# thomaspingel/neilpy

Hardware: AMD Instinct MI355X
Metric: Mcells/s through SMRF progressive_filter, 16384x16384 fp32 DEM (higher is better)
Workload: dtype f32

## Files before the change

include/smrf_hip.h:

```cpp
#ifndef SMRF_HIP_H
#define SMRF_HIP_H

#include <stddef.h>
#include <stdint.h>

#ifdef __cplusplus
extern "C" {
#endif

#define SMRF_ABI_VERSION 1

#if defined(__GNUC__)
#define SMRF_API __attribute__((visibility("default")))
#else
#define SMRF_API
#endif

#define SMRF_OK 0
#define SMRF_E_ARG (-1)
#define SMRF_E_HIP (-2)
#define SMRF_E_WORKSPACE (-3)
#define SMRF_E_RANGE (-4)
#define SMRF_E_UNSUPPORTED (-5)

// ... 46 lines not shown
SMRF_API size_t smrf_progressive_filter_workspace_bytes(int rows, int cols, int elem_size);
SMRF_API int smrf_progressive_filter_f32(const float* d_Z, int rows, int cols, const int32_t* h_windows,
                                const double* h_thresholds, int n_windows, uint8_t* d_mask,
                                uint8_t* d_when_dropped, void* d_workspace,
                                size_t workspace_bytes, int nan_aware, int impl, void* stream);
SMRF_API int smrf_progressive_filter_f64(const double* d_Z, int rows, int cols, const int32_t* h_windows,
                                const double* h_thresholds, int n_windows, uint8_t* d_mask,
                                uint8_t* d_when_dropped, void* d_workspace,
                                size_t workspace_bytes, int nan_aware, int impl, void* stream);

#define SMRF_ROUTE_TWO_PASS 0
#define SMRF_ROUTE_FUSED 1
#define SMRF_ROUTE_DIRECT 2
#define SMRF_ROUTE_COPY 3
#define SMRF_ROUTE_CHAIN 4
SMRF_API int smrf_progressive_filter_timed_f32(const float* d_Z, int rows, int cols, const int32_t* h_windows,
                                const double* h_thresholds, int n_windows, uint8_t* d_mask,
                                uint8_t* d_when_dropped, void* d_workspace, size_t workspace_bytes, int nan_aware,
                                int impl, void* stream, float* h_window_ms, int32_t* h_window_route);
SMRF_API int smrf_progressive_filter_timed_f64(const double* d_Z, int rows, int cols, const int32_t* h_windows,
                                const double* h_thresholds, int n_windows, uint8_t* d_mask,
                                uint8_t* d_when_dropped, void* d_workspace, size_t workspace_bytes, int nan_aware,
                                int impl, void* stream, float* h_window_ms, int32_t* h_window_route);

SMRF_API int smrf_count_nan_f32(const float* d_a, int64_t n, int64_t* h_count, void* stream);
SMRF_API int smrf_count_nan_f64(const double* d_a, int64_t n, int64_t* h_count, void* stream);

SMRF_API int smrf_points_extent_f64(const double* d_x, const double* d_y, int64_t n, double* h_out,
                           void* d_workspace, size_t workspace_bytes, void* stream);
SMRF_API int smrf_las_decode_xyz_f64(const uint8_t* d_records, int64_t npts, int record_length,
                            const double* h_scale_offset, double* d_x, double* d_y, double* d_z,
                            void* stream);
SMRF_API int smrf_affine_apply_f64(const double* d_x, const double* d_y, int64_t npts, const double* h_inv,
                          double* d_col, double* d_row, void* stream);
SMRF_API int smrf_grid_clear_u64(uint64_t* d_keys, int64_t ncells, void* stream);
SMRF_API int smrf_grid_bin_f64(const double* d_x, const double* d_y, const double* d_z, int64_t npts,
                      const double* h_inv, const double* h_filter, uint64_t* d_keys,
                      int rows_total, int cols, int row0, int rows_local, int is_max,
                      int64_t* d_n_outside, void* stream);
SMRF_API int smrf_grid_finalize_f64(const uint64_t* d_keys, double* d_grid, uint8_t* d_empty,
                           int64_t ncells, int is_max, void* stream);

SMRF_API int smrf_points_band_count_f64(const double* d_x, const double* d_y, int64_t npts, const double* h_inv,
                               int rows_total, int nbands, uint64_t* d_counts, void* stream);
SMRF_API int smrf_points_band_pack_f64(const double* d_x, const double* d_y, const double* d_z, int64_t npts,
                              const double* h_inv, int rows_total, int nbands, uint64_t* d_cursors,
// ... 92 lines not shown
```

neilpy_amd/_lib.py:

```python
import ctypes as C
import os

_HERE = os.path.dirname(os.path.abspath(__file__))
LIB_PATH = os.environ.get("NEILPY_AMD_LIB") or os.path.join(_HERE, "_lib", "libsmrf_hip.so")

IMPL_AUTO, IMPL_RING, IMPL_DIRECT = 0, 1, 2
ROUTE_TWO_PASS, ROUTE_FUSED, ROUTE_DIRECT, ROUTE_COPY, ROUTE_CHAIN = 0, 1, 2, 3, 4
RING_MAX_RADIUS = 64
TERRAIN_IMPL_AUTO, TERRAIN_IMPL_TILED, TERRAIN_IMPL_DIRECT = 0, 1, 2
TERRAIN_HALO_CAP = {"f32": 40, "f64": 24}
TERRAIN_OPENNESS, TERRAIN_SKYVIEW, TERRAIN_COUNT, TERRAIN_TERNARY = 0, 1, 2, 3
(SURFACE_SLOPE, SURFACE_ASPECT, SURFACE_HILLSHADE, SURFACE_HORN, SURFACE_LAPLACE, SURFACE_ESRI, SURFACE_ZT,
 SURFACE_EVANS, SURFACE_WG) = range(9)
SURFACE_OPT_RADIANS, SURFACE_OPT_DEGREES = 1, 2


class SmrfHipError(RuntimeError):
    pass


_p = C.c_void_p
_i = C.c_int
_i64 = C.c_int64
_d = C.c_double
_sz = C.c_size_t

SIGNATURES = {
    "smrf_abi_version": (_i, []),
    "smrf_last_error": (C.c_char_p, []),
    "smrf_device_count": (_i, []),
    "smrf_switches_reload": (None, []),
    "smrf_disk_filter_f32": (_i, [_p, _p, _i, _i, _i64, _i, _i, _i, _i, _i, _i, _i, _i, _p]),
    "smrf_disk_filter_f64": (_i, [_p, _p, _i, _i, _i64, _i, _i, _i, _i, _i, _i, _i, _i, _p]),
    "smrf_pf_dilate_flag_f32": (_i, [_p, _p, _p, _p, _p, _d, _i, _i, _i, _i64, _i, _i, _i, _i, _i, _i, _i, _p]),
    "smrf_pf_dilate_flag_f64": (_i, [_p, _p, _p, _p, _p, _d, _i, _i, _i, _i64, _i, _i, _i, _i, _i, _i, _i, _p]),
    "smrf_fused_open_supported": (_i, [_i, _i]),
    "smrf_pf_open_flag_f32": (_i, [_p, _p, _p, _p, _d, _i, _i, _i, _i64, _i, _i, _i, _i, _i, _p]),
    "smrf_pf_open_flag_f64": (_i, [_p, _p, _p, _p, _d, _i, _i, _i, _i64, _i, _i, _i, _i, _i, _p]),
    "smrf_pf_chain_length": (_i, [_i, _p, _i, _i64]),
    "smrf_pf_chain_flag_f32": (_i, [_p, _p, _p, _p, _p, _p, _p, _i, _i, _i, _i64, _i, _i, _i, _i, _p]),
    "smrf_pf_chain_flag_f64": (_i, [_p, _p, _p, _p, _p, _p, _p, _i, _i, _i, _i64, _i, _i, _i, _i, _p]),
    "smrf_progressive_filter_workspace_bytes": (_sz, [_i, _i, _i]),
    "smrf_progressive_filter_f32": (_i, [_p, _i, _i, _p, _p, _i, _p, _p, _p, _sz, _i, _i, _p]),
    "smrf_progressive_filter_f64": (_i, [_p, _i, _i, _p, _p, _i, _p, _p, _p, _sz, _i, _i, _p]),
    "smrf_progressive_filter_timed_f32": (_i, [_p, _i, _i, _p, _p, _i, _p, _p, _p, _sz, _i, _i, _p, _p, _p]),
    "smrf_progressive_filter_timed_f64": (_i, [_p, _i, _i, _p, _p, _i, _p, _p, _p, _sz, _i, _i, _p, _p, _p]),
    "smrf_count_nan_f32": (_i, [_p, _i64, C.POINTER(_i64), _p]),
    "smrf_count_nan_f64": (_i, [_p, _i64, C.POINTER(_i64), _p]),
    "smrf_points_extent_f64": (_i, [_p, _p, _i64, C.POINTER(_d), _p, _sz, _p]),
    "smrf_las_decode_xyz_f64": (_i, [_p, _i64, _i, C.POINTER(_d), _p, _p, _p, _p]),
    "smrf_affine_apply_f64": (_i, [_p, _p, _i64, C.POINTER(_d), _p, _p, _p]),
    "smrf_points_band_count_f64": (_i, [_p, _p, _i64, C.POINTER(_d), _i, _i, _p, _p]),
    "smrf_points_band_pack_f64": (_i, [_p, _p, _p, _i64, C.POINTER(_d), _i, _i, _p, _p, _p, _p, _p]),
    "smrf_grid_clear_u64": (_i, [_p, _i64, _p]),
    "smrf_grid_bin_f64": (_i, [_p, _p, _p, _i64, C.POINTER(_d), C.POINTER(_d), _p, _i, _i, _i, _i, _i, _p, _p]),
    "smrf_grid_finalize_f64": (_i, [_p, _p, _p, _i64, _i, _p]),
    "smrf_springs_workspace_bytes": (_sz, [_i, _i]),
    "smrf_springs_lsqr_f64": (_i, [_p, _i, _i, _d, _d, _d, _i64, C.POINTER(_i), C.POINTER(_i64),
                                   C.POINTER(_i64), _p, _sz, _p]),
    "smrf_fda_workspace_bytes": (_sz, [_i, _i]),
    "smrf_fda_lsqr_f64": (_i, [_p, _i, _i, _d, _d, _d, _i64, C.POINTER(_i), C.POINTER(_i64),
                               C.POINTER(_i64), _p, _sz, _p]),
    "smrf_fda_apply_f64": (_i, [_p, _i, _i, _p, _p, _p, _p, _p, _p, _p, _sz, _p]),
    "smrf_springs_band_workspace_bytes": (_sz, [_i, _i]),
    "smrf_springs_band_layout": (_i, [_i, _i, C.POINTER(_i64)]),
    "smrf_springs_band_begin": (_i, [_i, _i, _d, _d, _d, _i64, _p, _sz, _p]),
    "smrf_springs_band_phase": (_i, [_i, _p, _i, _i, _i, _i, _p, _sz, _p]),
    "smrf_springs_band_status": (_i, [_p, _i, _i, C.POINTER(_i), C.POINTER(_i64), C.POINTER(_i64), C.POINTER(_i), _p]),
    "smrf_gradient_slope_f64": (_i, [_p, _p, _i, _i, _d, _p]),
# ... 56 lines not shown
```

neilpy_amd/build.py:

```python
import argparse
import os
import shutil
import subprocess
import sys
from concurrent.futures import ThreadPoolExecutor

PKG = os.path.dirname(os.path.abspath(__file__))
ROOT = os.path.dirname(PKG)
CSRC = os.path.join(PKG, "csrc")
OBJ = os.path.join(PKG, "_build")
LIBDIR = os.path.join(PKG, "_lib")
LIB = os.path.join(LIBDIR, "libsmrf_hip.so")
RING_PARTS = 8

FLAGS = ["-std=c++20", "-O3", "--offload-arch=gfx950", "-fPIC", "-ffp-contract=off",
         "-fvisibility=hidden", "-Wall", "-Wno-unused-function",
         "-I" + os.path.join(ROOT, "include"), "-I" + CSRC]


def hipcc():
    exe = shutil.which("hipcc") or "/opt/rocm/bin/hipcc"
    if not os.path.exists(exe):
        raise RuntimeError("hipcc not found: libsmrf_hip cannot be built (there is no CPU fallback)")
    return exe


def units():
    out = [(n + ".o", os.path.join(CSRC, n + ".hip"), []) for n in ("core", "morph", "chain", "grid", "springs", "fda", "tail", "spline", "terrain", "surface")]
    for f64 in (0, 1):
        for p in range(RING_PARTS):
            out.append(("ring_%s_p%d.o" % ("f64" if f64 else "f32", p), os.path.join(CSRC, "ring_part.hip"),
                        ["-DPART=%d" % p, "-DSMRF_F64=%d" % f64]))
    return out


def newest_header():
    t = os.path.getmtime(os.path.join(ROOT, "include", "smrf_hip.h"))
    for f in os.listdir(CSRC):
        if f.endswith((".h", ".inc")):
            t = max(t, os.path.getmtime(os.path.join(CSRC, f)))
    return t


def build(jobs=None, force=False, verbose=True, variant=None, defs=()):
    global OBJ, LIB
    if variant:
        OBJ = os.path.join(PKG, "_build", "variant_" + variant)
        LIB = os.path.join(LIBDIR, "variants", variant + ".so")
        os.makedirs(os.path.dirname(LIB), exist_ok=True)
    os.makedirs(OBJ, exist_ok=True)
    os.makedirs(LIBDIR, exist_ok=True)
# ... 46 lines not shown
```

neilpy_amd/csrc/core.hip:

```cpp
#include <atomic>
#include <cstring>

#include "smrf_common.h"

namespace {
thread_local char g_err[512] = "";
}

namespace {
int env_int(const char* name, int dflt) {
  const char* v = getenv(name);
  return v && *v ? atoi(v) : dflt;
}
SmrfSwitches read_switches() {
  SmrfSwitches s;
  s.fused = env_int("SMRF_FUSED", 1);
  s.chain = env_int("SMRF_CHAIN", 1);
  s.nan_ride = env_int("SMRF_NAN_RIDE", 1);
  s.nt = env_int("SMRF_NT", -1);
  s.ring_seg = env_int("SMRF_RING_SEG", 0);
  s.ring_dual = env_int("SMRF_RING_DUAL", -1);
  s.ring_rounds = env_int("SMRF_RING_ROUNDS", 1);
  s.ring_slope = env_int("SMRF_RING_SLOPE", -1);
  s.seg_rule = env_int("SMRF_SEG_RULE", 0);
  s.xcd_remap = env_int("SMRF_XCD_REMAP", 1);
  s.fused_rounds = env_int("SMRF_FUSED_ROUNDS", 1);
  s.chain_rounds = env_int("SMRF_CHAIN_ROUNDS", 3);
  s.ring_debug = env_int("SMRF_RING_DEBUG", 0);
  return s;
}
std::atomic<const SmrfSwitches*> g_sw{new SmrfSwitches(read_switches())};
}

const SmrfSwitches& smrf_sw() { return *g_sw.load(std::memory_order_acquire); }

int smrf_fail(int code, const char* fmt, ...) {
  va_list ap;
  va_start(ap, fmt);
  vsnprintf(g_err, sizeof(g_err), fmt, ap);
  va_end(ap);
  return code;
}

extern "C" {

int smrf_abi_version(void) { return SMRF_ABI_VERSION; }

const char* smrf_last_error(void) { return g_err; }

void smrf_switches_reload(void) { g_sw.store(new SmrfSwitches(read_switches()), std::memory_order_release); }

// ... 11 lines not shown
```

neilpy_amd/csrc/morph.hip:

```cpp
#include <algorithm>
#include <cmath>
#include <cstdlib>
#include <cstring>
#include <vector>

#include "smrf_common.h"
#include "morph_chain.h"

namespace {

template <typename T>
__device__ __forceinline__ void flag_cell(const DiskArgs<T>& a, long long off, T lastval, T val) {
  const T diff = lastval - val;
  bool hit;
  if constexpr (sizeof(T) == 4) hit = diff > a.thr_lo;
  else hit = (double)diff > a.thr;
  if (a.dense) {
    a.mask[off] = hit ? 1 : 0;
    if (a.when != nullptr) a.when[off] = hit ? (uint8_t)a.widx : (uint8_t)0;
  } else if (hit) {
    a.mask[off] = 1;
    if (a.when != nullptr) a.when[off] = (uint8_t)a.widx;
  }
}
// ... 208 lines not shown
  if (!last || !opened || !mask || !radii || !thr || !widx) return smrf_fail(SMRF_E_ARG, "null pointer");
  if (n < 1 || n > 4) return smrf_fail(SMRF_E_ARG, "a chain has 1..4 windows (got %d)", n);
  const int pat = smrf_chain_match((int)sizeof(T), radii, n, 1ll << 62);
  if (pat < 0 || smrf_chain_length(pat) != n)
    return smrf_fail(SMRF_E_UNSUPPORTED, "no chained launch for these %d radii at this dtype (smrf_pf_chain_length tells)", n);
  DiskArgs<T> b{};
  b.in = last; b.out = opened; b.img_rows = img_rows; b.cols = cols; b.ld = ld;
  b.in_row0 = in_row0; b.in_rows = in_rows; b.out_row0 = out_row0; b.out_rows = out_rows;
  b.radius = smrf_chain_halo(pat);
  if (int rc = check_band(b)) return rc;
  if (b.radius >= img_rows) return smrf_fail(SMRF_E_UNSUPPORTED, "raster of %d rows is shorter than the chain's %d halo rows", img_rows, b.radius);
  ChainArgs<T> c{};
  c.in = last; c.out = opened; c.mask = mask; c.when = when;
  for (int k = 0; k < n; ++k) { c.thr[k] = thr[k]; c.widx[k] = widx[k]; }
  c.img_rows = img_rows; c.cols = cols; c.ld = ld;
  c.in_row0 = in_row0; c.in_rows = in_rows; c.out_row0 = out_row0; c.out_rows = out_rows;
  c.seg = smrf_sw().ring_seg;
  c.nt = nt_rule<T>(img_rows, cols);
  c.dense0 = 0;
  if constexpr (sizeof(T) == 4) return smrf_chain_f32(pat, c, (hipStream_t)stream);
  else return smrf_chain_f64(pat, c, (hipStream_t)stream);
}

template <typename T>
int progressive_filter_api(const T* Z, int rows, int cols, const int32_t* windows, const double* thr, int nwin,
                           uint8_t* mask, uint8_t* when, void* ws, size_t ws_bytes, int nan_aware, int impl,
                           void* stream_, float* h_window_ms = nullptr, int32_t* h_window_route = nullptr) {
  hipStream_t stream = (hipStream_t)stream_;
  if (!Z || !mask || (nwin > 0 && (!windows || !thr))) return smrf_fail(SMRF_E_ARG, "null pointer");
  if (rows < 1 || cols < 1 || nwin < 0) return smrf_fail(SMRF_E_ARG, "bad size");
  const size_t need = smrf_progressive_filter_workspace_bytes(rows, cols, (int)sizeof(T));
  if (ws_bytes < need || !ws) return smrf_fail(SMRF_E_WORKSPACE, "workspace %zu < %zu bytes", ws_bytes, need);
  for (int i = 0; i < nwin; ++i)
    if (windows[i] < 0) return smrf_fail(SMRF_E_ARG, "negative window %d", windows[i]);
  const size_t plane = (size_t)rows * cols;
  T* E = reinterpret_cast<T*>(ws);
  T* O[2] = {E + plane, E + 2 * plane};
  if (nwin == 0) {
    SMRF_HIP_CHECK(hipMemsetAsync(mask, 0, plane, stream));
    if (when) SMRF_HIP_CHECK(hipMemsetAsync(when, 0, plane, stream));
  }
  const int fuse_mode0 = smrf_sw().fused;
  const bool may_chain = nan_aware < 0 && nwin > 0 && fuse_mode0 != 0 && smrf_sw().chain != 0 &&
                         smrf_sw().nan_ride != 0 &&
                         (impl == SMRF_IMPL_AUTO || impl == SMRF_IMPL_RING);
  const int pat0 = may_chain ? smrf_chain_match((int)sizeof(T), windows, nwin, fuse_mode0 == 2 ? (1ll << 62) : (long long)plane) : -1;
  unsigned* d_nan = nullptr;
  if (nan_aware < 0) {
    if (pat0 >= 0 && smrf_chain_halo(pat0) < rows) {
      d_nan = reinterpret_cast<unsigned*>(E);
      SMRF_HIP_CHECK(hipMemsetAsync(d_nan, 0, sizeof(unsigned), stream));
      nan_aware = 0;
    } else {
      int64_t c = 0;
      if (int rc = count_nan_api<T>(Z, (int64_t)plane, &c, stream_)) return rc;
      nan_aware = c > 0;
    }
  }
  struct Events {
    std::vector<hipEvent_t> v;
// ... 1 lines not shown
  } evs;
  std::vector<hipEvent_t>& ev = evs.v;
  if (h_window_ms) {
    ev.assign((size_t)nwin + 1, nullptr);
    for (auto& e : ev) SMRF_HIP_CHECK(hipEventCreate(&e));
    SMRF_HIP_CHECK(hipEventRecord(ev[0], stream));
  }
  auto window_done = [&](int i, int route) -> int {
    if (h_window_route) h_window_route[i] = route;
    if (h_window_ms) SMRF_HIP_CHECK(hipEventRecord(ev[(size_t)i + 1], stream));
    return SMRF_OK;
  };
  auto finish = [&]() -> int {
    if (!h_window_ms) return SMRF_OK;
    hipError_t e = nwin > 0 ? hipEventSynchronize(ev[(size_t)nwin]) : hipSuccess;
    for (int i = 0; i < nwin && e == hipSuccess; ++i) e = hipEventElapsedTime(&h_window_ms[i], ev[(size_t)i], ev[(size_t)i + 1]);
    SMRF_HIP_CHECK(e);
    return SMRF_OK;
  };
  const T* last = Z;
  const int fuse_mode = smrf_sw().fused;
  const bool fuse_ok0 = (impl == SMRF_IMPL_AUTO || impl == SMRF_IMPL_RING) && fuse_mode != 0;
  const bool chain_ok0 = smrf_sw().chain != 0;
  int flip = 0;
  for (int i = 0; i < nwin;) {
    const int r = windows[i];
    T* opened = O[flip];
    flip ^= 1;
    const bool fuse_ok = !nan_aware && fuse_ok0;
    const bool chain_ok = fuse_ok && chain_ok0;
    const int pat = chain_ok ? smrf_chain_match((int)sizeof(T), windows + i, nwin - i, fuse_mode == 2 ? (1ll << 62) : (long long)plane) : -1;
    if (i == 0 && d_nan && pat != pat0) return smrf_fail(SMRF_E_HIP, "internal: first launch %d is not the one the NaN scan rides in (%d)", pat, pat0);
    if (pat >= 0 && smrf_chain_halo(pat) < rows) {
      const int len = smrf_chain_length(pat);
      ChainArgs<T> c{};
      c.in = last; c.out = opened; c.mask = mask; c.when = when;
      for (int k = 0; k < len; ++k) { c.thr[k] = thr[i + k]; c.widx[k] = i + k; }
      c.img_rows = rows; c.cols = cols; c.ld = cols;
      c.in_row0 = 0; c.in_rows = rows; c.out_row0 = 0; c.out_rows = rows;
      c.seg = smrf_sw().ring_seg;
      c.nt = nt_rule<T>(rows, cols);
      c.dense0 = i == 0;
      c.nan_flag = i == 0 ? d_nan : nullptr;
      int crc;
      if constexpr (sizeof(T) == 4) crc = smrf_chain_f32(pat, c, stream);
      else crc = smrf_chain_f64(pat, c, stream);
      if (crc) return crc;
      if (i == 0 && d_nan) {
        unsigned h = 0;
        SMRF_HIP_CHECK(hipMemcpyAsync(&h, d_nan, sizeof(h), hipMemcpyDeviceToHost, stream));
        SMRF_HIP_CHECK(hipStreamSynchronize(stream));
        d_nan = nullptr;
        if (h) {
          nan_aware = 1;
          flip = 0;
          last = Z;
          continue;
        }
      }
      if (nwin > 1) last = opened;
      for (int k = 0; k < len; ++k)
        if (int rc = window_done(i + k, SMRF_ROUTE_CHAIN + k)) return rc;
      i += len;
      continue;
    }
    if (fuse_ok && smrf_fused_radius((int)sizeof(T), r) && (r <= 8 || fuse_mode == 2 || plane >= ((size_t)20 << 20))) {
      if (int rc = open_flag_api<T>(last, opened, mask, when, thr[i], i, rows, cols, cols, 0, rows, 0, rows, r, stream_, i == 0)) return rc;
      if (nwin > 1) last = opened;
      if (int rc = window_done(i, SMRF_ROUTE_FUSED)) return rc;
      ++i;
      continue;
    }
    if (int rc = disk_filter_api<T>(last, E, rows, cols, cols, 0, rows, 0, rows, r, 0, nan_aware, impl, stream_)) return rc;
    if (int rc = dilate_flag_api<T>(E, last, opened, mask, when, thr[i], i, rows, cols, cols, 0, rows, 0, rows, r,
                                    nan_aware, impl, stream_, i == 0))
      return rc;
    if (nwin > 1) last = opened;
    const int eff = impl == SMRF_IMPL_AUTO ? (r <= SMRF_RING_MAX_RADIUS ? SMRF_IMPL_RING : SMRF_IMPL_DIRECT) : impl;
    if (int rc = window_done(i, r == 0 ? SMRF_ROUTE_COPY : eff == SMRF_IMPL_RING ? SMRF_ROUTE_TWO_PASS : SMRF_ROUTE_DIRECT)) return rc;
    ++i;
  }
  return finish();
}

}

extern "C" {

int smrf_disk_filter_f32(const float* d_in, float* d_out, int img_rows, int cols, int64_t ld, int in_row0,
                         int in_rows, int out_row0, int out_rows, int radius, int is_dilate, int nan_aware,
                         int impl, void* stream) {
  return disk_filter_api<float>(d_in, d_out, img_rows, cols, ld, in_row0, in_rows, out_row0, out_rows, radius,
                                is_dilate, nan_aware, impl, stream);
}
int smrf_disk_filter_f64(const double* d_in, double* d_out, int img_rows, int cols, int64_t ld, int in_row0,
                         int in_rows, int out_row0, int out_rows, int radius, int is_dilate, int nan_aware,
                         int impl, void* stream) {
  return disk_filter_api<double>(d_in, d_out, img_rows, cols, ld, in_row0, in_rows, out_row0, out_rows, radius,
                                 is_dilate, nan_aware, impl, stream);
}
int smrf_pf_dilate_flag_f32(const float* d_eroded, const float* d_last, float* d_opened, uint8_t* d_mask,
// ... 28 lines not shown
                               in_rows, out_row0, out_rows, radius, stream);
}
int smrf_pf_chain_length(int elem_size, const int32_t* h_radii, int n, int64_t raster_cells) {
  if (!h_radii || n < 1) return 0;
  const SmrfSwitches& sw = smrf_sw();
  if (sw.chain == 0 || sw.fused == 0) return 0;
  const int pat = smrf_chain_match(elem_size, h_radii, n, sw.fused == 2 ? (1ll << 62) : (long long)raster_cells);
  return pat < 0 ? 0 : smrf_chain_length(pat);
}
int smrf_pf_chain_flag_f32(const float* d_last, float* d_opened, uint8_t* d_mask, uint8_t* d_when_dropped,
                           const int32_t* h_radii, const double* h_thresholds, const int32_t* h_window_index, int n_windows,
                           int img_rows, int cols, int64_t ld, int in_row0, int in_rows, int out_row0, int out_rows,
                           void* stream) {
  return chain_flag_api<float>(d_last, d_opened, d_mask, d_when_dropped, h_radii, h_thresholds, h_window_index, n_windows,
                               img_rows, cols, ld, in_row0, in_rows, out_row0, out_rows, stream);
}
int smrf_pf_chain_flag_f64(const double* d_last, double* d_opened, uint8_t* d_mask, uint8_t* d_when_dropped,
                           const int32_t* h_radii, const double* h_thresholds, const int32_t* h_window_index, int n_windows,
                           int img_rows, int cols, int64_t ld, int in_row0, int in_rows, int out_row0, int out_rows,
                           void* stream) {
  return chain_flag_api<double>(d_last, d_opened, d_mask, d_when_dropped, h_radii, h_thresholds, h_window_index, n_windows,
                                img_rows, cols, ld, in_row0, in_rows, out_row0, out_rows, stream);
}
size_t smrf_progressive_filter_workspace_bytes(int rows, int cols, int elem_size) {
  return (size_t)3 * (size_t)rows * (size_t)cols * (size_t)elem_size;
}
int smrf_progressive_filter_f32(const float* d_Z, int rows, int cols, const int32_t* h_windows,
                                const double* h_thresholds, int n_windows, uint8_t* d_mask, uint8_t* d_when_dropped,
                                void* d_workspace, size_t workspace_bytes, int nan_aware, int impl, void* stream) {
  return progressive_filter_api<float>(d_Z, rows, cols, h_windows, h_thresholds, n_windows, d_mask, d_when_dropped,
                                       d_workspace, workspace_bytes, nan_aware, impl, stream);
}
int smrf_progressive_filter_f64(const double* d_Z, int rows, int cols, const int32_t* h_windows,
                                const double* h_thresholds, int n_windows, uint8_t* d_mask, uint8_t* d_when_dropped,
                                void* d_workspace, size_t workspace_bytes, int nan_aware, int impl, void* stream) {
  return progressive_filter_api<double>(d_Z, rows, cols, h_windows, h_thresholds, n_windows, d_mask, d_when_dropped,
                                        d_workspace, workspace_bytes, nan_aware, impl, stream);
}
int smrf_progressive_filter_timed_f32(const float* d_Z, int rows, int cols, const int32_t* h_windows,
                                      const double* h_thresholds, int n_windows, uint8_t* d_mask, uint8_t* d_when_dropped,
                                      void* d_workspace, size_t workspace_bytes, int nan_aware, int impl, void* stream,
                                      float* h_window_ms, int32_t* h_window_route) {
  if (!h_window_ms) return smrf_fail(SMRF_E_ARG, "null h_window_ms");
  return progressive_filter_api<float>(d_Z, rows, cols, h_windows, h_thresholds, n_windows, d_mask, d_when_dropped,
                                       d_workspace, workspace_bytes, nan_aware, impl, stream, h_window_ms, h_window_route);
}
// ... 17 lines not shown
```

neilpy_amd/csrc/smrf_common.h:

```cpp
#pragma once
#include <hip/hip_runtime.h>
#include <cstdarg>
#include <cstdint>
#include <cstdio>
#include <cstdlib>

#include "smrf_hip.h"

#define SMRF_HIDDEN __attribute__((visibility("hidden")))

SMRF_HIDDEN int smrf_fail(int code, const char* fmt, ...) __attribute__((format(printf, 2, 3)));

#define SMRF_HIP_CHECK(expr)                                                                  \
  do {                                                                                        \
    hipError_t e_ = (expr);                                                                   \
    if (e_ != hipSuccess)                                                                     \
      return smrf_fail(SMRF_E_HIP, "%s failed: %s (%s:%d)", #expr, hipGetErrorString(e_),     \
                       __FILE__, __LINE__);                                                   \
  } while (0)

#define SMRF_LAUNCH_CHECK() SMRF_HIP_CHECK(hipGetLastError())

__host__ __device__ inline int smrf_fold(int i, int n) {
  const int p2 = 2 * n;
  int p = i % p2;
  if (p < 0) p += p2;
  return p < n ? p : p2 - 1 - p;
}

struct SmrfSwitches {
  int fused;
  int chain;
  int nan_ride;
  int nt;
  int ring_seg;
  int ring_dual;
  int ring_rounds, fused_rounds, chain_rounds;
  int seg_rule;
  int xcd_remap;
  int ring_slope;
  int ring_debug;
};
SMRF_HIDDEN const SmrfSwitches& smrf_sw();

__host__ __device__ constexpr int smrf_isqrt(int v) {
  int r = 0;
  while ((long long)(r + 1) * (r + 1) <= v) ++r;
  return r;
}

inline float smrf_float_below(double t) {
  float f = (float)t;
  if ((double)f > t) f = __builtin_nextafterf(f, -__builtin_inff());
  return f;
}

#include "seg_rule.h"

template <typename T>
struct DiskArgs {
  const T* in;
  T* out;
  const T* last;
  uint8_t* mask;
// ... 2 lines not shown
  float thr_lo;
  int widx;
  int img_rows, cols;
  long long ld;
  int in_row0, in_rows, out_row0, out_rows;
  int radius;
  int nan_aware;
  int seg;
  int nt;
  int dense;
  int seg_cls;
  int seg_first[8], seg_row0[8], seg_len[8];
  int plain_tiles;
};

enum { SMRF_RING_ERODE = 0, SMRF_RING_DILATE = 1, SMRF_RING_FUSED_OPEN = 2 };
#ifndef SMRF_FUSED_MAX_RADIUS
#define SMRF_FUSED_MAX_RADIUS 14
#endif
constexpr bool smrf_fused_radius(int elem_size, int r) {
  if (r < 1 || r > SMRF_FUSED_MAX_RADIUS) return false;
  return elem_size == 4 ? (r != 9) : (r <= 6);
}
#define SMRF_RING_PARTS 8
#define SMRF_RING_DECL(P)                                                                     \
  SMRF_HIDDEN int smrf_ring_f32_p##P(const DiskArgs<float>&, int mode, hipStream_t);          \
  SMRF_HIDDEN int smrf_ring_f64_p##P(const DiskArgs<double>&, int mode, hipStream_t);
SMRF_RING_DECL(0) SMRF_RING_DECL(1) SMRF_RING_DECL(2) SMRF_RING_DECL(3)
SMRF_RING_DECL(4) SMRF_RING_DECL(5) SMRF_RING_DECL(6) SMRF_RING_DECL(7)
#undef SMRF_RING_DECL
```

Before: 4063.

## Add incremental erosion reusing previous window's erosion for consecutive radii

When consecutive windows differ by one radius and the previous window used the two-pass ring route, the new erosion is computed as a 3x3 min of the previous erosion combined with only the extra disk boundary offsets from a precomputed table. This replaces a full disk erosion with a much smaller stencil. It keeps three workspace planes rotating so the previous erosion stays available. It is adopted only for selected f32 radii via a per-radius table, and adds many template instantiations.

```diff
diff --git a/include/smrf_hip.h b/include/smrf_hip.h
--- a/include/smrf_hip.h
+++ b/include/smrf_hip.h
@@ -92,6 +92,8 @@
                                 const double* h_thresholds, int n_windows, uint8_t* d_mask,
                                 uint8_t* d_when_dropped, void* d_workspace, size_t workspace_bytes, int nan_aware,
                                 int impl, void* stream, float* h_window_ms, int32_t* h_window_route);
+
+SMRF_API int smrf_pf_ero_inc_windows(uint8_t* h_taken, int n);
 
 SMRF_API int smrf_count_nan_f32(const float* d_a, int64_t n, int64_t* h_count, void* stream);
 SMRF_API int smrf_count_nan_f64(const double* d_a, int64_t n, int64_t* h_count, void* stream);
diff --git a/neilpy_amd/_lib.py b/neilpy_amd/_lib.py
--- a/neilpy_amd/_lib.py
+++ b/neilpy_amd/_lib.py
@@ -45,6 +45,7 @@
     "smrf_progressive_filter_f64": (_i, [_p, _i, _i, _p, _p, _i, _p, _p, _p, _sz, _i, _i, _p]),
     "smrf_progressive_filter_timed_f32": (_i, [_p, _i, _i, _p, _p, _i, _p, _p, _p, _sz, _i, _i, _p, _p, _p]),
     "smrf_progressive_filter_timed_f64": (_i, [_p, _i, _i, _p, _p, _i, _p, _p, _p, _sz, _i, _i, _p, _p, _p]),
+    "smrf_pf_ero_inc_windows": (_i, [_p, _i]),
     "smrf_count_nan_f32": (_i, [_p, _i64, C.POINTER(_i64), _p]),
     "smrf_count_nan_f64": (_i, [_p, _i64, C.POINTER(_i64), _p]),
     "smrf_points_extent_f64": (_i, [_p, _p, _i64, C.POINTER(_d), _p, _sz, _p]),
diff --git a/neilpy_amd/build.py b/neilpy_amd/build.py
--- a/neilpy_amd/build.py
+++ b/neilpy_amd/build.py
@@ -26,7 +26,7 @@
 
 
 def units():
-    out = [(n + ".o", os.path.join(CSRC, n + ".hip"), []) for n in ("core", "morph", "chain", "grid", "springs", "fda", "tail", "spline", "terrain", "surface")]
+    out = [(n + ".o", os.path.join(CSRC, n + ".hip"), []) for n in ("core", "morph", "incero", "chain", "grid", "springs", "fda", "tail", "spline", "terrain", "surface")]
     for f64 in (0, 1):
         for p in range(RING_PARTS):
             out.append(("ring_%s_p%d.o" % ("f64" if f64 else "f32", p), os.path.join(CSRC, "ring_part.hip"),
diff --git a/neilpy_amd/csrc/core.hip b/neilpy_amd/csrc/core.hip
--- a/neilpy_amd/csrc/core.hip
+++ b/neilpy_amd/csrc/core.hip
@@ -27,6 +27,7 @@
   s.fused_rounds = env_int("SMRF_FUSED_ROUNDS", 1);
   s.chain_rounds = env_int("SMRF_CHAIN_ROUNDS", 3);
   s.ring_debug = env_int("SMRF_RING_DEBUG", 0);
+  s.ero_inc = env_int("SMRF_ERO_INC", 1);
   return s;
 }
 std::atomic<const SmrfSwitches*> g_sw{new SmrfSwitches(read_switches())};
diff --git a/neilpy_amd/csrc/ero_inc.inc b/neilpy_amd/csrc/ero_inc.inc
--- /dev/null
+++ b/neilpy_amd/csrc/ero_inc.inc
@@ -0,0 +1,69 @@
+struct EroIncPair { signed char dy; unsigned char dx; };
+struct EroIncTab { int n, reach; EroIncPair p[28]; };
+inline constexpr EroIncTab kEroInc[65] = {
+    {0, 0, {}},
+    {0, 0, {}},
+    {0, 0, {}},
+    {2, 2, {{-2, 2}, {2, 2}}},
+    {0, 0, {}},
+    {4, 4, {{-4, 3}, {-3, 4}, {3, 4}, {4, 3}}},
+    {0, 0, {}},
+    {0, 0, {}},
+    {4, 6, {{-6, 5}, {-5, 6}, {5, 6}, {6, 5}}},
+    {4, 8, {{-8, 4}, {-4, 8}, {4, 8}, {8, 4}}},
+    {6, 8, {{-8, 6}, {-7, 7}, {-6, 8}, {6, 8}, {7, 7}, {8, 6}}},
+    {0, 0, {}},
+    {0, 0, {}},
+    {10, 12, {{-12, 5}, {-10, 8}, {-9, 9}, {-8, 10}, {-5, 12}, {5, 12}, {8, 10}, {9, 9}, {10, 8}, {12, 5}}},
+    {4, 12, {{-12, 7}, {-7, 12}, {7, 12}, {12, 7}}},
+    {8, 12, {{-12, 9}, {-11, 10}, {-10, 11}, {-9, 12}, {9, 12}, {10, 11}, {11, 10}, {12, 9}}},
+    {0, 0, {}},
+    {6, 15, {{-15, 8}, {-12, 12}, {-8, 15}, {8, 15}, {12, 12}, {15, 8}}},
+    {4, 14, {{-14, 11}, {-11, 14}, {11, 14}, {14, 11}}},
+    {8, 18, {{-18, 6}, {-16, 10}, {-10, 16}, {-6, 18}, {6, 18}, {10, 16}, {16, 10}, {18, 6}}},
+    {10, 16, {{-16, 12}, {-15, 13}, {-14, 14}, {-13, 15}, {-12, 16}, {12, 16}, {13, 15}, {14, 14}, {15, 13}, {16, 12}}},
+    {0, 0, {}},
+    {12, 20, {{-20, 9}, {-19, 11}, {-16, 15}, {-15, 16}, {-11, 19}, {-9, 20}, {9, 20}, {11, 19}, {15, 16}, {16, 15}, {19, 11}, {20, 9}}},
+    {4, 18, {{-18, 14}, {-14, 18}, {14, 18}, {18, 14}}},
+    {4, 20, {{-20, 13}, {-13, 20}, {13, 20}, {20, 13}}},
+    {16, 24, {{-24, 7}, {-20, 15}, {-19, 16}, {-18, 17}, {-17, 18}, {-16, 19}, {-15, 20}, {-7, 24}, {7, 24}, {15, 20}, {16, 19}, {17, 18}, {18, 17}, {19, 16}, {20, 15}, {24, 7}}},
+    {8, 24, {{-24, 10}, {-23, 12}, {-12, 23}, {-10, 24}, {10, 24}, {12, 23}, {23, 12}, {24, 10}}},
+    {10, 23, {{-23, 14}, {-20, 18}, {-19, 19}, {-18, 20}, {-14, 23}, {14, 23}, {18, 20}, {19, 19}, {20, 18}, {23, 14}}},
+    {4, 22, {{-22, 17}, {-17, 22}, {17, 22}, {22, 17}}},
+    {8, 24, {{-24, 16}, {-21, 20}, {-20, 21}, {-16, 24}, {16, 24}, {20, 21}, {21, 20}, {24, 16}}},
+    {12, 27, {{-27, 13}, {-24, 18}, {-23, 19}, {-19, 23}, {-18, 24}, {-13, 27}, {13, 27}, {18, 24}, {19, 23}, {23, 19}, {24, 18}, {27, 13}}},
+    {4, 27, {{-27, 15}, {-15, 27}, {15, 27}, {27, 15}}},
+    {16, 30, {{-30, 11}, {-27, 17}, {-24, 21}, {-23, 22}, {-22, 23}, {-21, 24}, {-17, 27}, {-11, 30}, {11, 30}, {17, 27}, {21, 24}, {22, 23}, {23, 22}, {24, 21}, {27, 17}, {30, 11}}},
+    {8, 32, {{-32, 8}, {-26, 20}, {-20, 26}, {-8, 32}, {8, 32}, {20, 26}, {26, 20}, {32, 8}}},
+    {14, 30, {{-30, 16}, {-28, 19}, {-25, 23}, {-24, 24}, {-23, 25}, {-19, 28}, {-16, 30}, {16, 30}, {19, 28}, {23, 25}, {24, 24}, {25, 23}, {28, 19}, {30, 16}}},
+    {16, 32, {{-32, 14}, {-30, 18}, {-28, 21}, {-27, 22}, {-22, 27}, {-21, 28}, {-18, 30}, {-14, 32}, {14, 32}, {18, 30}, {21, 28}, {22, 27}, {27, 22}, {28, 21}, {30, 18}, {32, 14}}},
+    {0, 0, {}},
+    {18, 35, {{-35, 12}, {-31, 20}, {-28, 24}, {-27, 25}, {-26, 26}, {-25, 27}, {-24, 28}, {-20, 31}, {-12, 35}, {12, 35}, {20, 31}, {24, 28}, {25, 27}, {26, 26}, {27, 25}, {28, 24}, {31, 20}, {35, 12}}},
+    {4, 30, {{-30, 23}, {-23, 30}, {23, 30}, {30, 23}}},
+    {24, 36, {{-36, 15}, {-35, 17}, {-34, 19}, {-32, 22}, {-29, 26}, {-28, 27}, {-27, 28}, {-26, 29}, {-22, 32}, {-19, 34}, {-17, 35}, {-15, 36}, {15, 36}, {17, 35}, {19, 34}, {22, 32}, {26, 29}, {27, 28}, {28, 27}, {29, 26}, {32, 22}, {34, 19}, {35, 17}, {36, 15}}},
+    {12, 34, {{-34, 21}, {-32, 24}, {-31, 25}, {-25, 31}, {-24, 32}, {-21, 34}, {21, 34}, {24, 32}, {25, 31}, {31, 25}, {32, 24}, {34, 21}}},
+    {4, 40, {{-40, 9}, {-9, 40}, {9, 40}, {40, 9}}},
+    {16, 35, {{-35, 23}, {-32, 27}, {-31, 28}, {-30, 29}, {-29, 30}, {-28, 31}, {-27, 32}, {-23, 35}, {23, 35}, {27, 32}, {28, 31}, {29, 30}, {30, 29}, {31, 28}, {32, 27}, {35, 23}}},
+    {12, 39, {{-39, 18}, {-38, 20}, {-34, 26}, {-26, 34}, {-20, 38}, {-18, 39}, {18, 39}, {20, 38}, {26, 34}, {34, 26}, {38, 20}, {39, 18}}},
+    {22, 42, {{-42, 13}, {-38, 22}, {-36, 25}, {-33, 29}, {-32, 30}, {-31, 31}, {-30, 32}, {-29, 33}, {-25, 36}, {-22, 38}, {-13, 42}, {13, 42}, {22, 38}, {25, 36}, {29, 33}, {30, 32}, {31, 31}, {32, 30}, {33, 29}, {36, 25}, {38, 22}, {42, 13}}},
+    {16, 42, {{-42, 16}, {-38, 24}, {-36, 27}, {-35, 28}, {-28, 35}, {-27, 36}, {-24, 38}, {-16, 42}, {16, 42}, {24, 38}, {27, 36}, {28, 35}, {35, 28}, {36, 27}, {38, 24}, {42, 16}}},
+    {4, 33, {{-33, 32}, {-32, 33}, {32, 33}, {33, 32}}},
+    {16, 42, {{-42, 21}, {-39, 26}, {-36, 30}, {-35, 31}, {-31, 35}, {-30, 36}, {-26, 39}, {-21, 42}, {21, 42}, {26, 39}, {30, 36}, {31, 35}, {35, 31}, {36, 30}, {39, 26}, {42, 21}}},
+    {12, 44, {{-44, 19}, {-42, 23}, {-38, 29}, {-29, 38}, {-23, 42}, {-19, 44}, {19, 44}, {23, 42}, {29, 38}, {38, 29}, {42, 23}, {44, 19}}},
+    {20, 42, {{-42, 25}, {-40, 28}, {-37, 32}, {-36, 33}, {-35, 34}, {-34, 35}, {-33, 36}, {-32, 37}, {-28, 40}, {-25, 42}, {25, 42}, {28, 40}, {32, 37}, {33, 36}, {34, 35}, {35, 34}, {36, 33}, {37, 32}, {40, 28}, {42, 25}}},
+    {20, 48, {{-48, 14}, {-47, 17}, {-42, 27}, {-40, 30}, {-39, 31}, {-31, 39}, {-30, 40}, {-27, 42}, {-17, 47}, {-14, 48}, {14, 48}, {17, 47}, {27, 42}, {30, 40}, {31, 39}, {39, 31}, {40, 30}, {42, 27}, {47, 17}, {48, 14}}},
+    {22, 50, {{-50, 10}, {-46, 22}, {-45, 24}, {-38, 34}, {-37, 35}, {-36, 36}, {-35, 37}, {-34, 38}, {-24, 45}, {-22, 46}, {-10, 50}, {10, 50}, {22, 46}, {24, 45}, {34, 38}, {35, 37}, {36, 36}, {37, 35}, {38, 34}, {45, 24}, {46, 22}, {50, 10}}},
+    {16, 48, {{-48, 20}, {-45, 26}, {-43, 29}, {-40, 33}, {-33, 40}, {-29, 43}, {-26, 45}, {-20, 48}, {20, 48}, {26, 45}, {29, 43}, {33, 40}, {40, 33}, {43, 29}, {45, 26}, {48, 20}}},
+    {8, 45, {{-45, 28}, {-42, 32}, {-32, 42}, {-28, 45}, {28, 45}, {32, 42}, {42, 32}, {45, 28}}},
+    {18, 44, {{-44, 31}, {-41, 35}, {-40, 36}, {-39, 37}, {-38, 38}, {-37, 39}, {-36, 40}, {-35, 41}, {-31, 44}, {31, 44}, {35, 41}, {36, 40}, {37, 39}, {38, 38}, {39, 37}, {40, 36}, {41, 35}, {44, 31}}},
+    {12, 46, {{-46, 30}, {-44, 33}, {-43, 34}, {-34, 43}, {-33, 44}, {-30, 46}, {30, 46}, {33, 44}, {34, 43}, {43, 34}, {44, 33}, {46, 30}}},
+    {28, 53, {{-53, 18}, {-51, 23}, {-50, 25}, {-49, 27}, {-42, 37}, {-41, 38}, {-40, 39}, {-39, 40}, {-38, 41}, {-37, 42}, {-27, 49}, {-25, 50}, {-23, 51}, {-18, 53}, {18, 53}, {23, 51}, {25, 50}, {27, 49}, {37, 42}, {38, 41}, {39, 40}, {40, 39}, {41, 38}, {42, 37}, {49, 27}, {50, 25}, {51, 23}, {53, 18}}},
+    {12, 49, {{-49, 29}, {-47, 32}, {-44, 36}, {-36, 44}, {-32, 47}, {-29, 49}, {29, 49}, {32, 47}, {36, 44}, {44, 36}, {47, 32}, {49, 29}}},
+    {22, 56, {{-56, 15}, {-54, 21}, {-49, 31}, {-46, 35}, {-42, 40}, {-41, 41}, {-40, 42}, {-35, 46}, {-31, 49}, {-21, 54}, {-15, 56}, {15, 56}, {21, 54}, {31, 49}, {35, 46}, {40, 42}, {41, 41}, {42, 40}, {46, 35}, {49, 31}, {54, 21}, {56, 15}}},
+    {12, 48, {{-48, 34}, {-45, 38}, {-44, 39}, {-39, 44}, {-38, 45}, {-34, 48}, {34, 48}, {38, 45}, {39, 44}, {44, 39}, {45, 38}, {48, 34}}},
+    {20, 54, {{-54, 26}, {-53, 28}, {-50, 33}, {-48, 36}, {-47, 37}, {-37, 47}, {-36, 48}, {-33, 50}, {-28, 53}, {-26, 54}, {26, 54}, {28, 53}, {33, 50}, {36, 48}, {37, 47}, {47, 37}, {48, 36}, {50, 33}, {53, 28}, {54, 26}}},
+    {26, 60, {{-60, 11}, {-56, 24}, {-53, 30}, {-46, 40}, {-45, 41}, {-44, 42}, {-43, 43}, {-42, 44}, {-41, 45}, {-40, 46}, {-30, 53}, {-24, 56}, {-11, 60}, {11, 60}, {24, 56}, {30, 53}, {40, 46}, {41, 45}, {42, 44}, {43, 43}, {44, 42}, {45, 41}, {46, 40}, {53, 30}, {56, 24}, {60, 11}}},
+    {16, 59, {{-59, 19}, {-53, 32}, {-51, 35}, {-48, 39}, {-39, 48}, {-35, 51}, {-32, 53}, {-19, 59}, {19, 59}, {32, 53}, {35, 51}, {39, 48}, {48, 39}, {51, 35}, {53, 32}, {59, 19}}},
+    {20, 59, {{-59, 22}, {-53, 34}, {-50, 38}, {-46, 43}, {-45, 44}, {-44, 45}, {-43, 46}, {-38, 50}, {-34, 53}, {-22, 59}, {22, 59}, {34, 53}, {38, 50}, {43, 46}, {44, 45}, {45, 44}, {46, 43}, {50, 38}, {53, 34}, {59, 22}}},
+    {20, 58, {{-58, 27}, {-57, 29}, {-52, 37}, {-49, 41}, {-48, 42}, {-42, 48}, {-41, 49}, {-37, 52}, {-29, 57}, {-27, 58}, {27, 58}, {29, 57}, {37, 52}, {41, 49}, {42, 48}, {48, 42}, {49, 41}, {52, 37}, {57, 29}, {58, 27}}},
+};
diff --git a/neilpy_amd/csrc/ero_inc_adopt.inc b/neilpy_amd/csrc/ero_inc_adopt.inc
--- /dev/null
+++ b/neilpy_amd/csrc/ero_inc_adopt.inc
@@ -0,0 +1,5 @@
+inline constexpr unsigned char kEroIncAdoptF32[65] = {
+    0, 0, 0, 0, 0, 0, 0, 0, 0, 0, 0, 0, 0, 0, 0, 0, 0,
+    0, 0, 0, 0, 1, 0, 0, 0, 0, 0, 0, 1, 1, 0, 1, 0, 0,
+    1, 0, 1, 0, 1, 0, 1, 1, 1, 1, 0, 1, 1, 1, 1, 1, 1,
+    0, 0, 0, 0, 0, 0, 0, 0, 0, 0, 0, 0, 0, 0};
diff --git a/neilpy_amd/csrc/incero.hip b/neilpy_amd/csrc/incero.hip
--- /dev/null
+++ b/neilpy_amd/csrc/incero.hip
@@ -0,0 +1,27 @@
+#include "morph_incero.h"
+
+namespace {
+template <int R>
+int launch_r(const smrf::IncEroArgs<float>& a, hipStream_t s) { return smrf::inc_erode_launch<float, R>(a, s); }
+}
+
+bool smrf_inc_erode_has(int elem_size, int radius) {
+  return elem_size == 4 && radius >= SMRF_INCERO_MIN_RADIUS && radius <= SMRF_INCERO_MAX_RADIUS;
+}
+bool smrf_inc_erode_adopted(int elem_size, int radius) {
+  return smrf_inc_erode_has(elem_size, radius) && smrf::kEroIncAdoptF32[radius] != 0;
+}
+
+int smrf_inc_erode_f32(const float* e_prev, const float* last, float* out, int rows, int cols, long long ld, int radius, int nt,
+                       hipStream_t s) {
+  smrf::IncEroArgs<float> a{};
+  a.e_prev = e_prev; a.last = last; a.out = out; a.rows = rows; a.cols = cols; a.ld = ld; a.nt = nt;
+  a.seg = smrf_sw().ring_seg;
+#define SMRF_INCERO_CASE(R) case R: return launch_r<R>(a, s);
+#define SMRF_INCERO_CASE4(R) SMRF_INCERO_CASE(R) SMRF_INCERO_CASE(R + 1) SMRF_INCERO_CASE(R + 2) SMRF_INCERO_CASE(R + 3)
+#define SMRF_INCERO_CASE16(R) SMRF_INCERO_CASE4(R) SMRF_INCERO_CASE4(R + 4) SMRF_INCERO_CASE4(R + 8) SMRF_INCERO_CASE4(R + 12)
+  switch (radius) {
+    SMRF_INCERO_CASE16(16) SMRF_INCERO_CASE16(32) SMRF_INCERO_CASE16(48) SMRF_INCERO_CASE(64)
+    default: return smrf_fail(SMRF_E_UNSUPPORTED, "no incremental erosion kernel for radius %d", radius);
+  }
+}
diff --git a/neilpy_amd/csrc/morph.hip b/neilpy_amd/csrc/morph.hip
--- a/neilpy_amd/csrc/morph.hip
+++ b/neilpy_amd/csrc/morph.hip
@@ -254,6 +254,8 @@
   else return smrf_chain_f64(pat, c, (hipStream_t)stream);
 }
 
+thread_local std::vector<uint8_t> g_ero_inc_taken;
+
 template <typename T>
 int progressive_filter_api(const T* Z, int rows, int cols, const int32_t* windows, const double* thr, int nwin,
                            uint8_t* mask, uint8_t* when, void* ws, size_t ws_bytes, int nan_aware, int impl,
@@ -267,7 +269,10 @@
     if (windows[i] < 0) return smrf_fail(SMRF_E_ARG, "negative window %d", windows[i]);
   const size_t plane = (size_t)rows * cols;
   T* E = reinterpret_cast<T*>(ws);
-  T* O[2] = {E + plane, E + 2 * plane};
+  T* P[3] = {E, E + plane, E + 2 * plane};
+  int pe = 0, pl = -1;
+  auto spare = [&]() { for (int k = 0; k < 3; ++k) if (k != pe && k != pl) return k; return 0; };
+  g_ero_inc_taken.assign((size_t)nwin, 0);
   if (nwin == 0) {
     SMRF_HIP_CHECK(hipMemsetAsync(mask, 0, plane, stream));
     if (when) SMRF_HIP_CHECK(hipMemsetAsync(when, 0, plane, stream));
@@ -315,11 +320,12 @@
   const int fuse_mode = smrf_sw().fused;
   const bool fuse_ok0 = (impl == SMRF_IMPL_AUTO || impl == SMRF_IMPL_RING) && fuse_mode != 0;
   const bool chain_ok0 = smrf_sw().chain != 0;
-  int flip = 0;
+  const int inc_mode = smrf_sw().ero_inc;
+  int ring_two_pass_at = -2;
   for (int i = 0; i < nwin;) {
     const int r = windows[i];
-    T* opened = O[flip];
-    flip ^= 1;
+    const int po = spare();
+    T* opened = P[po];
     const bool fuse_ok = !nan_aware && fuse_ok0;
     const bool chain_ok = fuse_ok && chain_ok0;
     const int pat = chain_ok ? smrf_chain_match((int)sizeof(T), windows + i, nwin - i, fuse_mode == 2 ? (1ll << 62) : (long long)plane) : -1;
@@ -346,12 +352,12 @@
         d_nan = nullptr;
         if (h) {
           nan_aware = 1;
-          flip = 0;
+          pe = 0; pl = -1;
           last = Z;
           continue;
         }
       }
-      if (nwin > 1) last = opened;
+      if (nwin > 1) { last = opened; pl = po; }
       for (int k = 0; k < len; ++k)
         if (int rc = window_done(i + k, SMRF_ROUTE_CHAIN + k)) return rc;
       i += len;
@@ -359,17 +365,37 @@
     }
     if (fuse_ok && smrf_fused_radius((int)sizeof(T), r) && (r <= 8 || fuse_mode == 2 || plane >= ((size_t)20 << 20))) {
       if (int rc = open_flag_api<T>(last, opened, mask, when, thr[i], i, rows, cols, cols, 0, rows, 0, rows, r, stream_, i == 0)) return rc;
-      if (nwin > 1) last = opened;
+      if (nwin > 1) { last = opened; pl = po; }
       if (int rc = window_done(i, SMRF_ROUTE_FUSED)) return rc;
       ++i;
       continue;
     }
-    if (int rc = disk_filter_api<T>(last, E, rows, cols, cols, 0, rows, 0, rows, r, 0, nan_aware, impl, stream_)) return rc;
-    if (int rc = dilate_flag_api<T>(E, last, opened, mask, when, thr[i], i, rows, cols, cols, 0, rows, 0, rows, r,
-                                    nan_aware, impl, stream_, i == 0))
-      return rc;
-    if (nwin > 1) last = opened;
     const int eff = impl == SMRF_IMPL_AUTO ? (r <= SMRF_RING_MAX_RADIUS ? SMRF_IMPL_RING : SMRF_IMPL_DIRECT) : impl;
+    const bool inc = inc_mode != 0 && !nan_aware && eff == SMRF_IMPL_RING && i > 0 && ring_two_pass_at == i - 1 && pl >= 0 &&
+                     r == windows[i - 1] + 1 && smrf_inc_erode_has((int)sizeof(T), r) &&
+                     (inc_mode == 2 || smrf_inc_erode_adopted((int)sizeof(T), r));
+    if (inc) {
+      if constexpr (sizeof(T) == 4) {
+        if (int rc = smrf_inc_erode_f32(P[pe], last, P[po], rows, cols, cols, r, nt_rule<T>(rows, cols), stream)) return rc;
+      } else {
+        return smrf_fail(SMRF_E_HIP, "internal: no incremental erosion at this dtype");
+      }
+      opened = P[pe];
+      if (int rc = dilate_flag_api<T>(P[po], last, opened, mask, when, thr[i], i, rows, cols, cols, 0, rows, 0, rows, r,
+                                      nan_aware, impl, stream_, 0))
+        return rc;
+      last = opened;
+      pl = pe;
+      pe = po;
+      g_ero_inc_taken[(size_t)i] = 1;
+    } else {
+      if (int rc = disk_filter_api<T>(last, P[pe], rows, cols, cols, 0, rows, 0, rows, r, 0, nan_aware, impl, stream_)) return rc;
+      if (int rc = dilate_flag_api<T>(P[pe], last, opened, mask, when, thr[i], i, rows, cols, cols, 0, rows, 0, rows, r,
+                                      nan_aware, impl, stream_, i == 0))
+        return rc;
+      if (nwin > 1) { last = opened; pl = po; }
+    }
+    if (eff == SMRF_IMPL_RING && r >= 1) ring_two_pass_at = i;
     if (int rc = window_done(i, r == 0 ? SMRF_ROUTE_COPY : eff == SMRF_IMPL_RING ? SMRF_ROUTE_TWO_PASS : SMRF_ROUTE_DIRECT)) return rc;
     ++i;
   }
@@ -444,6 +470,12 @@
   return chain_flag_api<double>(d_last, d_opened, d_mask, d_when_dropped, h_radii, h_thresholds, h_window_index, n_windows,
                                 img_rows, cols, ld, in_row0, in_rows, out_row0, out_rows, stream);
 }
+int smrf_pf_ero_inc_windows(uint8_t* h_taken, int n) {
+  if (!h_taken || n < 0) return smrf_fail(SMRF_E_ARG, "null h_taken");
+  const int have = (int)g_ero_inc_taken.size();
+  for (int i = 0; i < n; ++i) h_taken[i] = i < have ? g_ero_inc_taken[(size_t)i] : 0;
+  return have;
+}
 size_t smrf_progressive_filter_workspace_bytes(int rows, int cols, int elem_size) {
   return (size_t)3 * (size_t)rows * (size_t)cols * (size_t)elem_size;
 }
diff --git a/neilpy_amd/csrc/morph_incero.h b/neilpy_amd/csrc/morph_incero.h
--- /dev/null
+++ b/neilpy_amd/csrc/morph_incero.h
@@ -0,0 +1,209 @@
+#pragma once
+#include "morph_ring.h"
+
+namespace smrf {
+
+#include "ero_inc.inc"
+#include "ero_inc_adopt.inc"
+
+#define SMRF_INCERO_MIN_RADIUS 16
+#define SMRF_INCERO_MAX_RADIUS 64
+
+template <typename T>
+struct IncEroArgs {
+  const T* e_prev;
+  const T* last;
+  T* out;
+  int rows, cols;
+  long long ld;
+  int seg;
+  int nt;
+  int plain_tiles;
+};
+
+template <int R>
+struct IncEroCfg {
+  static constexpr int N = kEroInc[R].n;
+  static constexpr int DY = kEroInc[R].reach;
+  static constexpr int TW = 256, NP = 4, ROWS = 2 * NP;
+  static constexpr int W = TW + 2 * DY;
+  static constexpr int NPOS = (W + TW - 1) / TW;
+  static constexpr int NACC = 2 * DY + ROWS;
+  static constexpr int G = 4;
+  static constexpr int NJ = NP * N;
+  static constexpr int NG = (NJ + G - 1) / G;
+  static constexpr int gsize(int g) { const int n = NJ - g * G; return n < 0 ? 0 : n > G ? G : n; }
+  static constexpr int dy(int k) { return kEroInc[R].p[k].dy; }
+  static constexpr int dx(int k) { return kEroInc[R].p[k].dx; }
+  static constexpr int DELTA = (ROWS - (2 * DY) % ROWS) % ROWS;
+  static constexpr int LDS_CELLS = N > 0 ? 2 * NP * W : 1;
+};
+
+template <typename T, int R>
+__global__ __launch_bounds__(256) void inc_erode_kernel(const IncEroArgs<T> a) {
+  using C = IncEroCfg<R>;
+  using T2 = typename Vec2<T>::type;
+  constexpr int N = C::N, DY = C::DY, TW = C::TW, NP = C::NP, ROWS = C::ROWS, W = C::W, NPOS = C::NPOS, NACC = C::NACC, G = C::G;
+  __shared__ T2 L[C::LDS_CELLS];
+  const int tid = threadIdx.x;
+  int bx = blockIdx.x, by = blockIdx.y;
+  if (a.plain_tiles) {
+  } else if ((gridDim.x & 7) == 0) {
+    const int id = blockIdx.y * gridDim.x + blockIdx.x, per = gridDim.x >> 3;
+    const int xcd = id & 7, slot = id >> 3;
+    bx = xcd * per + slot % per;
+    by = slot / per;
+  } else if (gridDim.x > 8) {
+    const int total = gridDim.x * gridDim.y, id = blockIdx.y * gridDim.x + blockIdx.x;
+    const int xcd = id & 7, slot = id >> 3, q = total >> 3, rem = total & 7;
+    const int t = xcd * q + (xcd < rem ? xcd : rem) + slot;
+    bx = t / (int)gridDim.y;
+    by = t % (int)gridDim.y;
+  }
+  const int x0 = bx * TW, x = x0 + tid;
+  const int ys = by * a.seg, ye = min(a.rows, ys + a.seg);
+  if (ys >= ye) return;
+  const int xc = x < a.cols ? x : a.cols - 1;
+  const int xl = smrf_fold(xc - 1, a.cols), xr = smrf_fold(xc + 1, a.cols);
+  int cpos[NPOS];
+  bool act[NPOS];
+#pragma unroll
+  for (int i = 0; i < NPOS; ++i) {
+    act[i] = tid + i * TW < W;
+    cpos[i] = smrf_fold(x0 - DY + tid + (act[i] ? i * TW : 0), a.cols);
+  }
+  T acc[NACC];
+#pragma unroll
+  for (int i = 0; i < NACC; ++i) acc[i] = ident<T>(false);
+
+  int o0 = ys - 2 * DY - C::DELTA;
+  const int nb = (ye - o0 + ROWS - 1) / ROWS;
+  RowFold rf(o0 + DY, a.rows);
+  T2 pf[NP][NPOS];
+  auto prefetch = [&]() {
+#pragma unroll
+    for (int p = 0; p < NP; ++p) {
+      const T* ra = a.last + (long long)rf.at(2 * p) * a.ld;
+      const T* rb = a.last + (long long)rf.at(2 * p + 1) * a.ld;
+#pragma unroll
+      for (int i = 0; i < NPOS; ++i)
+        if (i < NPOS - 1 || act[i]) { pf[p][i].x = ra[cpos[i]]; pf[p][i].y = rb[cpos[i]]; }
+    }
+    rf.advance(ROWS);
+  };
+  if constexpr (N > 0) prefetch();
+
+  for (int b = 0; b < nb; ++b, o0 += ROWS) {
+    const unsigned lds_b = (unsigned)(size_t)(__attribute__((address_space(3))) void*)(L + (b & 1) * NP * W + tid);
+    if constexpr (N > 0) {
+#pragma unroll
+      for (int p = 0; p < NP; ++p)
+#pragma unroll
+        for (int i = 0; i < NPOS; ++i)
+          if (i < NPOS - 1 || act[i]) lds_write2(lds_b + (unsigned)((p * W + i * TW) * (int)sizeof(T2)), pf[p][i]);
+      lds_wait<0>();
+      __syncthreads();
+      if (b + 1 < nb) prefetch();
+    }
+    const bool store = o0 >= ys;
+    T ec[ROWS + 2], el[ROWS], er[ROWS];
+    if (store) {
+      RowFold rfe(o0 - 1, a.rows);
+#pragma unroll
+      for (int j = 0; j < ROWS + 2; ++j) {
+        const T* row = a.e_prev + (long long)rfe.at(j) * a.ld;
+        ec[j] = row[xc];
+        if (j >= 1 && j <= ROWS) { el[j - 1] = row[xl]; er[j - 1] = row[xr]; }
+      }
+    }
+    if constexpr (N > 0) {
+      T2 rd[2 * G][2];
+      auto issue = [&]<int J>(std::integral_constant<int, J>) {
+        constexpr int p = J / N, k = J % N;
+        constexpr int offl = (p * W + DY - C::dx(k)) * (int)sizeof(T2), offr = (p * W + DY + C::dx(k)) * (int)sizeof(T2);
+        rd[J % (2 * G)][0] = lds_read2<offl>(lds_b, T());
+        rd[J % (2 * G)][1] = lds_read2<offr>(lds_b, T());
+      };
+      auto apply = [&]<int J>(std::integral_constant<int, J>) {
+        constexpr int p = J / N, k = J % N, s = 2 * p - C::dy(k) + DY;
+        static_assert(s >= 0 && s + 1 < NACC, "slot outside the ring");
+        op3_acc<false>(acc[s], rd[J % (2 * G)][0].x, rd[J % (2 * G)][1].x);
+        op3_acc<false>(acc[s + 1], rd[J % (2 * G)][0].y, rd[J % (2 * G)][1].y);
+      };
+      auto issue_group = [&]<int Gi>(std::integral_constant<int, Gi>) {
+        [&]<int... I>(std::integer_sequence<int, I...>) {
+          (issue(std::integral_constant<int, Gi * G + I>{}), ...);
+        }(std::make_integer_sequence<int, C::gsize(Gi)>{});
+      };
+      auto apply_group = [&]<int Gi>(std::integral_constant<int, Gi>) {
+        [&]<int... I>(std::integer_sequence<int, I...>) {
+          (apply(std::integral_constant<int, Gi * G + I>{}), ...);
+        }(std::make_integer_sequence<int, C::gsize(Gi)>{});
+      };
+      issue_group(std::integral_constant<int, 0>{});
+      [&]<int... Gi>(std::integer_sequence<int, Gi...>) {
+        (([&] {
+           if constexpr (Gi + 1 < C::NG) {
+             issue_group(std::integral_constant<int, Gi + 1>{});
+             lds_wait<2 * C::gsize(Gi + 1)>();
+           } else {
+             lds_wait<0>();
+           }
+           apply_group(std::integral_constant<int, Gi>{});
+         }()),
+         ...);
+      }(std::make_integer_sequence<int, C::NG>{});
+    }
+    if (store) {
+#pragma unroll
+      for (int j = 0; j < ROWS; ++j) {
+        T m = op3<false>(ec[j + 1], el[j], er[j]);
+        m = op3<false>(m, ec[j], ec[j + 2]);
+        if constexpr (N > 0) m = op2<false>(m, acc[j]);
+        const int o = o0 + j;
+        if (o < ye && x < a.cols) smrf_store_out(a.out + (long long)o * a.ld + x, m, a.nt);
+      }
+    }
+    if constexpr (N > 0) {
+#pragma unroll
+      for (int s = 0; s < NACC - ROWS; ++s) acc[s] = acc[s + ROWS];
+#pragma unroll
+      for (int s = NACC - ROWS; s < NACC; ++s) acc[s] = ident<T>(false);
+    }
+  }
+}
+
+template <typename T, int R>
+int inc_erode_launch(const IncEroArgs<T>& a_in, hipStream_t stream) {
+  using C = IncEroCfg<R>;
+  auto kern = inc_erode_kernel<T, R>;
+  static int resident_of[64] = {0};
+  int dev = 0;
+  SMRF_HIP_CHECK(hipGetDevice(&dev));
+  if (dev < 0 || dev >= 64) return smrf_fail(SMRF_E_UNSUPPORTED, "device index %d out of range", dev);
+  int resident = __atomic_load_n(&resident_of[dev], __ATOMIC_ACQUIRE);
+  if (resident == 0) {
+    int nb = 0;
+    SMRF_HIP_CHECK(hipOccupancyMaxActiveBlocksPerMultiprocessor(&nb, reinterpret_cast<const void*>(kern), C::TW, 0));
+    resident = std::max(1, nb);
+    __atomic_store_n(&resident_of[dev], resident, __ATOMIC_RELEASE);
+    if (smrf_sw().ring_debug)
+      fprintf(stderr, "smrf inc erode: R=%d pairs=%d reach=%d LDS=%zu, %d workgroups/CU resident\n", R, C::N, C::DY,
+              C::LDS_CELLS * 2 * sizeof(T), resident);
+  }
+  IncEroArgs<T> a = a_in;
+  const int strips = (a.cols + C::TW - 1) / C::TW;
+  if (a.seg <= 0) {
+    const int nseg = smrf_pick_nseg(a.rows, strips, resident, smrf_sw().ring_rounds, 2 * C::DY + C::DELTA, C::ROWS,
+                                    std::max(32, 4 * C::DY), smrf_sw().seg_rule);
+    a.seg = (a.rows + nseg - 1) / nseg;
+  }
+  a.seg = ((a.seg + C::ROWS - 1) / C::ROWS) * C::ROWS;
+  a.plain_tiles = smrf_sw().xcd_remap ? 0 : 1;
+  dim3 grid(strips, (a.rows + a.seg - 1) / a.seg);
+  hipLaunchKernelGGL(kern, grid, dim3(C::TW), 0, stream, a);
+  SMRF_LAUNCH_CHECK();
+  return SMRF_OK;
+}
+
+}
diff --git a/neilpy_amd/csrc/smrf_common.h b/neilpy_amd/csrc/smrf_common.h
--- a/neilpy_amd/csrc/smrf_common.h
+++ b/neilpy_amd/csrc/smrf_common.h
@@ -40,6 +40,7 @@
   int xcd_remap;
   int ring_slope;
   int ring_debug;
+  int ero_inc;
 };
 SMRF_HIDDEN const SmrfSwitches& smrf_sw();
 
@@ -88,6 +89,10 @@
   if (r < 1 || r > SMRF_FUSED_MAX_RADIUS) return false;
   return elem_size == 4 ? (r != 9) : (r <= 6);
 }
+SMRF_HIDDEN bool smrf_inc_erode_has(int elem_size, int radius);
+SMRF_HIDDEN bool smrf_inc_erode_adopted(int elem_size, int radius);
+SMRF_HIDDEN int smrf_inc_erode_f32(const float* e_prev, const float* last, float* out, int rows, int cols, long long ld,
+                                   int radius, int nt, hipStream_t s);
 #define SMRF_RING_PARTS 8
 #define SMRF_RING_DECL(P)                                                                     \
   SMRF_HIDDEN int smrf_ring_f32_p##P(const DiskArgs<float>&, int mode, hipStream_t);          \
```

After: 4225, median of 6. +4.0%, better.
